# Avirup221/Multimodal-Hierarchical-CNN-for-Sun-Salutation-Pose-Classification

Measured on AMD Instinct MI355X. Metric: images/sec fwd+bwd QuadtreeCNN 224x224 bs256, higher is better.
Workload: dtype bf16; 1 GPU; QuadtreeCNN (ResNet-18 layer3, 2x2 split, 47-feat fusion) train step fwd+bwd+Adam, all parameters trainable; Adam(lr 1e-4, wd 1e-4) by the package's FusedAdam (csrc/pack.hip); global_batch=256, per_gpu_batch=256, image=3x224x224, num_classes=12, parallelism=dp1

## Files before the change

include/qtcnn.h:

```cpp
#ifndef QTCNN_H_
#define QTCNN_H_

#include <stddef.h>
#include <stdint.h>

#ifdef __cplusplus
extern "C" {
#endif

typedef enum qt_status {
  QT_OK = 0,
  QT_ERR_INVALID_ARG = -1,
  QT_ERR_LAUNCH = -2,
  QT_ERR_UNSUPPORTED = -3
} qt_status;

typedef enum qt_dtype { QT_F32 = 0, QT_BF16 = 1 } qt_dtype;

int qt_version(void);
const char* qt_last_error(void);

enum { QT_CONV_FWD = 0, QT_CONV_DGRAD = 1 };

typedef struct qt_conv_desc {
// ... 274 lines not shown
void qt_plan_destroy(qt_plan* plan);
int qt_plan_num_tensors(const qt_plan* plan);
const char* qt_plan_tensor_name(const qt_plan* plan, int i);
int qt_plan_tensor_kind(const qt_plan* plan, int i);
int qt_plan_tensor_shape(const qt_plan* plan, int i, int* dims4);
size_t qt_plan_workspace_bytes(const qt_plan* plan);
int qt_plan_find_buffer(const qt_plan* plan, const char* name, size_t* offset);
int qt_plan_profile_begin(qt_plan* plan);
int qt_plan_profile_end(qt_plan* plan, double* flops3, double* ms3, int* launches3);
int qt_plan_profile_bytes(const qt_plan* plan, double* bytes3);
int qt_plan_side_fence(qt_plan* plan, void* waiting_stream);
int qt_plan_init_workspace(qt_plan* plan, void* workspace, void* stream);
int qt_plan_pack_weights(qt_plan* plan, void* workspace, void* const* tensors, int for_backward, void* stream);
int qt_plan_adam_step(qt_plan* plan, void* workspace, void* const* tensors, float* const* grads, float* const* exp_avg,
                      float* const* exp_avg_sq, const qt_adam_desc* adam, int for_backward, void* stream);
int qt_plan_forward(qt_plan* plan, void* workspace, void* const* tensors, const float* image, const float* numerical,
                    float* logits, int batch, int training, unsigned long long seed, void* stream);
int qt_plan_backward(qt_plan* plan, void* workspace, void* const* tensors, float* const* grads, const float* numerical,
                     const float* dlogits, int phases, void* stream);
int qt_plan_backward_dx(qt_plan* plan, void* workspace, void* const* tensors, float* const* grads,
                        const float* numerical, const float* dlogits, int phases, float* dimage, void* stream);

#ifdef __cplusplus
}
#endif
#endif
```

multimodal-hierarchical-cnn-for-sun-salutation-pose-classification_amd/csrc/pack.hip:

```cpp
#include <math.h>
#include <string.h>

#include "qt_common.h"

namespace {

template <typename T> __device__ __forceinline__ T qt_from_f32(float v);
template <> __device__ __forceinline__ float qt_from_f32<float>(float v) { return v; }
template <> __device__ __forceinline__ bf16_t qt_from_f32<bf16_t>(float v) { return (bf16_t)v; }

template <typename T>
__global__ void pack_stem_input_kernel(const float* __restrict__ img, T* __restrict__ dst, int batch) {
  constexpr int PH = QT_STEM_PAD_H, PW = QT_STEM_PAD_W;
  const long long total = (long long)batch * PH * PW;
  for (long long i = blockIdx.x * (long long)blockDim.x + threadIdx.x; i < total;
       i += (long long)gridDim.x * blockDim.x) {
    const int pw = (int)(i % PW);
    const int ph = (int)((i / PW) % PH);
    const int n = (int)(i / ((long long)PW * PH));
    const int h = ph - 3, w = pw - 3;
    float v[4] = {0.f, 0.f, 0.f, 0.f};
    if ((unsigned)h < 224u && (unsigned)w < 224u) {
      const float* s = img + (long long)n * 3 * 224 * 224 + h * 224 + w;
      v[0] = s[0];
// ... 21 lines not shown
    const int o = (int)(idx / ((long long)I * taps));
    const float v = w[((long long)o * I + i) * taps + tap];
    if (fwd) fwd[idx] = qt_from_f32<T>(v);
    if (dgrad) dgrad[((long long)i * taps + tap) * O + o] = qt_from_f32<T>(v);
  }
}

struct AdamScalars {
  float lr, b1, b2, eps, wd;
  float step_size;
  float inv_sqrt_bc2;
  float grad_scale;
  int enabled;
};
__device__ __forceinline__ float adam_update(float p, float g, float& m, float& v, const AdamScalars& h) {
  g = g * h.grad_scale + h.wd * p;
  m = h.b1 * m + (1.f - h.b1) * g;
  v = h.b2 * v + (1.f - h.b2) * g * g;
  const float denom = sqrtf(v) * h.inv_sqrt_bc2 + h.eps;
  return p - h.step_size * (m / denom);
}

constexpr int PK_MAX_ITEMS = 32;
struct PackBatchArgs {
  AdamScalars adam;
  const float* g[PK_MAX_ITEMS];
  float* m[PK_MAX_ITEMS];
  float* v[PK_MAX_ITEMS];
  const float* w[PK_MAX_ITEMS];
  void* fwd[PK_MAX_ITEMS];
  void* dgrad[PK_MAX_ITEMS];
  int O[PK_MAX_ITEMS], I[PK_MAX_ITEMS];
  unsigned char k[PK_MAX_ITEMS], s2[PK_MAX_ITEMS];
  int first_block[PK_MAX_ITEMS + 1];
  int n;
};

template <typename T> struct PackPair;
template <> struct PackPair<float> {
  static __device__ __forceinline__ void store(float* p, float a, float b) { *reinterpret_cast<float2*>(p) = make_float2(a, b); }
};
template <> struct PackPair<bf16_t> {
  static __device__ __forceinline__ void store(bf16_t* p, float a, float b) {
    typedef __attribute__((ext_vector_type(2))) __bf16 bf16x2;
    bf16x2 v = {(bf16_t)a, (bf16_t)b};
    *reinterpret_cast<bf16x2*>(p) = v;
  }
};

template <typename T, int TAPS, int TO, int TI>
__device__ __forceinline__ void pack_tile(float* tile, const float* w, T* __restrict__ fwd, T* __restrict__ dg,
                                          int O, int I, int o0, int i0, int s2, const AdamScalars& adam,
                                          const float* __restrict__ g, float* m, float* v) {
  constexpr int RUN = TI * TAPS, S = RUN + 1, TOTAL = TO * RUN;
  for (int e = threadIdx.x; e < TOTAL; e += 256) {
    const int o = e / RUN, r = e - o * RUN;
    const long long idx = ((long long)(o0 + o) * I + i0) * TAPS + r;
    float pv = w[idx];
    if (adam.enabled) {
      float mv = m[idx], vv = v[idx];
      pv = adam_update(pv, g[idx], mv, vv, adam);
      m[idx] = mv;
      v[idx] = vv;
      const_cast<float*>(w)[idx] = pv;
    }
    tile[o * S + r] = pv;
  }
  __syncthreads();
  if (fwd) {
    for (int e = threadIdx.x; e < TOTAL / 2; e += 256) {
      const int i = (e % (TI / 2)) * 2, ot = e / (TI / 2);
      const int o = ot / TAPS, tap = ot - o * TAPS;
      const float* t = tile + o * S + i * TAPS + tap;
      PackPair<T>::store(fwd + ((long long)(o0 + o) * TAPS + tap) * I + i0 + i, t[0], t[TAPS]);
    }
  }
  if (dg) {
    for (int e = threadIdx.x; e < TOTAL / 2; e += 256) {
      const int o = (e % (TO / 2)) * 2, it2 = e / (TO / 2);
      const int i = it2 / TAPS, tap = it2 - i * TAPS;
      const float* t = tile + o * S + i * TAPS + tap;
      long long dst;
      if (TAPS == 1 && s2 == 4) {
        dst = ((long long)(i0 + i) * 5 + 4) * O + o0 + o;
      } else if (TAPS == 1 || !s2) {
        dst = ((long long)(i0 + i) * TAPS + tap) * O + o0 + o;
      } else {
        const int kh = tap / 3, kw = tap - kh * 3;
        const int ph = kh != 1, pw = kw != 1;
        const int th = ph ? (kh == 2 ? 0 : 1) : 0, tw = pw ? (kw == 2 ? 0 : 1) : 0;
        const int nh = ph ? 2 : 1, nw = pw ? 2 : 1;
        const int cls = ph * 2 + pw;
        const long long IO = (long long)I * O;
        const long long base = cls == 0 ? 0 : (cls == 1 ? IO : (cls == 2 ? 3 * IO : 5 * IO));
        dst = base + ((long long)(i0 + i) * (nh * nw) + th * nw + tw) * O + o0 + o;
        if (s2 == 2) dst = (((long long)cls * I + i0 + i) * 4 + th * 2 + tw) * O + o0 + o;
        if (s2 == 3) dst = (((long long)cls * I + i0 + i) * 5 + th * 2 + tw) * O + o0 + o;
      }
      PackPair<T>::store(dg + dst, t[0], t[S]);
    }
  }
}

constexpr int PK_T1 = 64;

template <typename T>
__global__ __launch_bounds__(256) void pack_weights_batched_kernel(PackBatchArgs a) {
  __shared__ float tile[32 * (32 * 9 + 1)];
  static_assert(PK_T1 * (PK_T1 + 1) <= 32 * (32 * 9 + 1), "1x1 tile fits the 3x3 tile's LDS");
  int it = 0;
  while (it + 1 < a.n && (int)blockIdx.x >= a.first_block[it + 1]) ++it;
  const int O = a.O[it], I = a.I[it];
  const int b = blockIdx.x - a.first_block[it];
  T* fwd = static_cast<T*>(a.fwd[it]);
  T* dg = static_cast<T*>(a.dgrad[it]);
  if (a.k[it] == 1) {
    const int tiles_i = I / PK_T1;
    pack_tile<T, 1, PK_T1, PK_T1>(tile, a.w[it], fwd, dg, O, I, (b / tiles_i) * PK_T1, (b % tiles_i) * PK_T1, (int)a.s2[it], a.adam,
                                  a.g[it], a.m[it], a.v[it]);
  } else {
    const int tiles_i = I >> 5;
    pack_tile<T, 9, 32, 32>(tile, a.w[it], fwd, dg, O, I, (b / tiles_i) << 5, (b % tiles_i) << 5, (int)a.s2[it], a.adam,
                            a.g[it], a.m[it], a.v[it]);
  }
}

constexpr int AD_MAX_ITEMS = 48, AD_CHUNK = 4096;
struct AdamBatchArgs {
  AdamScalars adam;
  float* p[AD_MAX_ITEMS];
  const float* g[AD_MAX_ITEMS];
  float* m[AD_MAX_ITEMS];
  float* v[AD_MAX_ITEMS];
  long long numel[AD_MAX_ITEMS];
  int first_block[AD_MAX_ITEMS + 1];
  int n;
};
__global__ __launch_bounds__(256) void adam_multi_kernel(AdamBatchArgs a) {
// ... 181 lines not shown
  QT_CHECK_ARG(items && n > 0 && n <= PK_MAX_ITEMS, "qt_pack_weights_batched: 1..%d items", PK_MAX_ITEMS);
  QT_CHECK_ARG(dtype == QT_F32 || dtype == QT_BF16, "qt_pack_weights_batched: bad dtype %d", dtype);
  PackBatchArgs a;
  memset(&a, 0, sizeof(a));
  if (opt) {
    if (int st = make_adam_scalars(adam, &a.adam)) return st;
  }
  int blocks = 0;
  for (int j = 0; j < n; ++j) {
    const qt_pack_item& q = items[j];
    const int te = q.k == 1 ? PK_T1 : 32;
    QT_CHECK_ARG(q.w_oihw && (q.w_fwd || q.w_dgrad) && (q.k == 1 || q.k == 3) && q.O > 0 && q.I > 0 && q.O % te == 0 &&
                     q.I % te == 0,
                 "qt_pack_weights_batched: item %d: O=%d I=%d must be multiples of %d for k=%d (k in {1,3})", j, q.O, q.I,
                 te, q.k);
    a.w[j] = q.w_oihw; a.fwd[j] = q.w_fwd; a.dgrad[j] = q.w_dgrad;
    if (opt) {
      const qt_adam_item& u = opt[j];
      QT_CHECK_ARG(u.param == q.w_oihw && u.grad && u.exp_avg && u.exp_avg_sq &&
                       u.numel == (long long)q.O * q.I * q.k * q.k,
                   "qt_adam_pack_weights_batched: item %d: optimizer state does not match the weight", j);
      a.g[j] = u.grad; a.m[j] = u.exp_avg; a.v[j] = u.exp_avg_sq;
    }
    a.O[j] = q.O; a.I[j] = q.I; a.k[j] = (unsigned char)q.k; a.s2[j] = (unsigned char)((q.stride2_dgrad >= 2 && q.stride2_dgrad <= 4) ? q.stride2_dgrad : (q.stride2_dgrad ? 1 : 0));
    QT_CHECK_ARG(q.stride2_dgrad != 4 || q.k == 1, "qt_pack_weights_batched: item %d: stride2_dgrad = 4 is for 1x1 filters", j);
    QT_CHECK_ARG(q.stride2_dgrad != 3 || q.k == 3, "qt_pack_weights_batched: item %d: stride2_dgrad = 3 is for 3x3 filters", j);
    a.first_block[j] = blocks;
    blocks += (q.O / te) * (q.I / te);
  }
  a.first_block[n] = blocks;
  a.n = n;
  hipStream_t s = static_cast<hipStream_t>(stream);
  if (dtype == QT_F32)
    hipLaunchKernelGGL(pack_weights_batched_kernel<float>, dim3(blocks), dim3(256), 0, s, a);
  else
    hipLaunchKernelGGL(pack_weights_batched_kernel<bf16_t>, dim3(blocks), dim3(256), 0, s, a);
  QT_CHECK_LAUNCH();
  return QT_OK;
}

extern "C" int qt_pack_dgrad_s2(int dtype, const float* w_oihw, void* dst, int O, int I, int k, long long* class_offset,
                                int* class_kh, int* class_kw, void* stream) {
  QT_CHECK_ARG(w_oihw && O > 0 && I > 0 && (k == 1 || k == 3), "qt_pack_dgrad_s2: bad argument");
// ... 73 lines not shown
```

multimodal-hierarchical-cnn-for-sun-salutation-pose-classification_amd/csrc/plan.hip:

```cpp
#include <stdlib.h>
#include <string.h>

#include <algorithm>
#include <string>
#include <vector>

#include "qt_common.h"

static bool merged_s2_enabled() {
  static int v = -1;
  if (v < 0) {
    const char* e = getenv("QTCNN_S2_DGRAD_MERGED");
    v = e ? (atoi(e) != 0) : 1;
  }
  return v != 0;
}

static bool ds_slot_enabled() {
  static int v = -1;
  if (v < 0) {
    const char* e = getenv("QTCNN_DS_SLOT");
    v = e ? (atoi(e) != 0) : 1;
  }
  return v != 0;
// ... 71 lines not shown
  size_t stats_bn2 = 0, stats_ds = 0, stats_bn1 = 0;
  size_t dw_begin = 0, dw_end = 0;
  size_t lin_ws = 0, lin_ws_bytes = 0;
  size_t wgrad_part = 0, wgrad_part_bytes = 0;
  bool packed_fwd = false, packed_bwd = false;
  unsigned long long packed_sig = 0;
  bool dw_dirty = true;
  int bwd_rows_bn2 = 0;
  struct Timed { hipEvent_t a, b; double flops; double bytes; int kind; };
  double last_profile_bytes[3] = {0, 0, 0};
  bool profiling = false;
  std::vector<Timed> timed;
  bool use_side = true;
  hipStream_t side = nullptr;
  hipEvent_t ev_fork = nullptr, ev_join = nullptr;
  int last_batch = 0, last_training = 0;
  unsigned long long last_seed = 0;

  int add_tensor(const std::string& name, int kind, std::initializer_list<int> shape) {
    TensorInfo t;
    t.name = name;
    t.kind = kind;
    t.ndim = (int)shape.size();
    int i = 0;
    for (int s : shape) t.shape[i++] = s;
    for (; i < 4; ++i) t.shape[i] = 1;
    tensors.push_back(t);
    return (int)tensors.size() - 1;
  }
  int add_bn(const std::string& prefix, int C) {
// ... 590 lines not shown
}
size_t dgrad_operand(const qt_plan* p, const ConvL& c) {
  return (c.k == 1 && c.slot_conv >= 0) ? p->convs[c.slot_conv].w_dgrad : c.w_dgrad;
}

unsigned long long weight_sig(const qt_plan* p, void* const* T) {
  unsigned long long h = 1469598103934665603ull;
  auto mix = [&](const void* ptr) { h = (h ^ (unsigned long long)(uintptr_t)ptr) * 1099511628211ull; };
  for (const ConvL& c : p->convs) mix(T[c.w]);
  mix(T[p->cls0.w]);
  return h;
}

int pack_weights(qt_plan* p, void* workspace, void* const* T, int for_backward, void* stream) {
  Exec e{p, static_cast<unsigned char*>(workspace), T, stream, p->d.batch, p->d.dtype};
  std::vector<qt_pack_item> items;
  auto add = [&](const float* w, void* fwd, void* dgrad, int O, int I, int k, int s2) {
    qt_pack_item q;
    q.w_oihw = w; q.w_fwd = fwd; q.w_dgrad = dgrad; q.O = O; q.I = I; q.k = k; q.stride2_dgrad = s2;
    items.push_back(q);
  };
  if (p->has_image) {
    for (size_t i = 0; i < p->convs.size(); ++i) {
      const ConvL& c = p->convs[i];
      if (i == 0)
        e.run(qt_pack_stem_weight(e.dt, e.tf(c.w), e.at(c.w_fwd), e.stem_taps(), stream));
      else
        add(e.tf(c.w), e.at(c.w_fwd), for_backward ? e.at(dgrad_operand(p, c)) : nullptr, c.cout, c.cin, c.k, dgrad_layout(c));
    }
  }
  if (!p->lstm)
    add(e.tf(p->cls0.w), e.at(p->cls0.w_fwd), for_backward ? e.at(p->cls0.w_dgrad) : nullptr, p->cls0.out, p->cls0.in, 1,
        false);
  for (size_t j = 0; j < items.size() && e.ok(); j += 32)
    e.run(qt_pack_weights_batched(e.dt, items.data() + j, (int)std::min<size_t>(32, items.size() - j), stream));
  p->packed_fwd = e.ok();
  p->packed_bwd = e.ok() && for_backward != 0;
  p->packed_sig = weight_sig(p, T);
  return e.status;
}

int adam_step(qt_plan* p, void* workspace, void* const* T, float* const* G, float* const* M1, float* const* M2,
              const qt_adam_desc* adam, int for_backward, void* stream) {
  Exec e{p, static_cast<unsigned char*>(workspace), T, stream, p->d.batch, p->d.dtype};
  std::vector<bool> fused(p->tensors.size(), false);
  std::vector<qt_pack_item> upd_items, pack_items;
  std::vector<qt_adam_item> upd_state, plain;
  auto numel_of = [&](int idx) {
    long long n = 1;
    for (int d = 0; d < p->tensors[idx].ndim; ++d) n *= p->tensors[idx].shape[d];
    return n;
  };
  auto add = [&](int widx, void* fwd, void* dgrad, int O, int I, int k, int s2) -> int {
    qt_pack_item q;
    q.w_oihw = e.tf(widx); q.w_fwd = fwd; q.w_dgrad = dgrad; q.O = O; q.I = I; q.k = k; q.stride2_dgrad = s2;
    if (G[widx]) {
      QT_CHECK_ARG(M1[widx] && M2[widx], "qt_plan_adam_step: %s has a gradient but no optimizer state",
                   p->tensors[widx].name.c_str());
      qt_adam_item u;
      u.param = e.tf(widx); u.grad = G[widx]; u.exp_avg = M1[widx]; u.exp_avg_sq = M2[widx]; u.numel = numel_of(widx);
      upd_items.push_back(q);
      upd_state.push_back(u);
// ... 5 lines not shown
  };
  if (p->has_image)
    for (size_t i = 1; i < p->convs.size(); ++i) {
      const ConvL& c = p->convs[i];
      if (int st = add(c.w, e.at(c.w_fwd), for_backward ? e.at(dgrad_operand(p, c)) : nullptr, c.cout, c.cin, c.k, dgrad_layout(c))) return st;
    }
  if (!p->lstm)
    if (int st = add(p->cls0.w, e.at(p->cls0.w_fwd), for_backward ? e.at(p->cls0.w_dgrad) : nullptr, p->cls0.out, p->cls0.in, 1, false))
      return st;
  for (size_t i = 0; i < p->tensors.size(); ++i) {
    if (p->tensors[i].kind != 0 || fused[i] || !G[i]) continue;
    QT_CHECK_ARG(T[i] && M1[i] && M2[i], "qt_plan_adam_step: %s has a gradient but no parameter / optimizer state",
                 p->tensors[i].name.c_str());
    qt_adam_item u;
    u.param = e.tf((int)i); u.grad = G[i]; u.exp_avg = M1[i]; u.exp_avg_sq = M2[i]; u.numel = numel_of((int)i);
    plain.push_back(u);
  }
  if (!plain.empty()) e.run(qt_adam_multi(plain.data(), (int)plain.size(), adam, stream));
  if (p->has_image)
    e.run(qt_pack_stem_weight(e.dt, e.tf(p->convs[0].w), e.at(p->convs[0].w_fwd), e.stem_taps(), stream));
  for (size_t j = 0; j < upd_items.size() && e.ok(); j += 32) {
    const int cnt = (int)std::min<size_t>(32, upd_items.size() - j);
    e.run(qt_adam_pack_weights_batched(e.dt, upd_items.data() + j, upd_state.data() + j, adam, cnt, stream));
  }
  const unsigned long long sig = weight_sig(p, T);
  const bool frozen_current = p->packed_fwd && (!for_backward || p->packed_bwd) && p->packed_sig == sig;
  if (!frozen_current)
    for (size_t j = 0; j < pack_items.size() && e.ok(); j += 32)
      e.run(qt_pack_weights_batched(e.dt, pack_items.data() + j, (int)std::min<size_t>(32, pack_items.size() - j), stream));
  p->packed_fwd = e.ok();
  p->packed_bwd = e.ok() && (for_backward != 0);
  p->packed_sig = sig;
  return e.status;
}

int forward(qt_plan* p, void* workspace, void* const* T, const float* image, const float* numerical, float* logits,
            int batch, int training, unsigned long long seed, void* stream) {
  Exec e{p, static_cast<unsigned char*>(workspace), T, stream, batch, p->d.dtype};
  e.setup_side();
  const int dt = e.dt;
  const bool tr = training == 1;
  const bool unf = training != 0;
  hipStream_t hs = static_cast<hipStream_t>(stream);
  auto quad_branch = [&]() {
    const ConvL& cq = p->convs[p->quad_conv];
    e.igemm(e.quad_desc(QT_CONV_FWD), e.at(p->blocks[5].out), e.at(cq.w_fwd), e.at(p->q), nullptr, e.tf(cq.bias),
            nullptr, nullptr, nullptr, 1);
    e.run(qt_quad_pool(dt, e.at(p->q), e.at(p->fused), batch, p->fused_ld, 512, e.stream));
  };
  auto mlp_branch = [&]() {
    qt_gemm_small_desc g;
    memset(&g, 0, sizeof(g));
    g.M = batch; g.N = p->mlp0.out; g.K = p->mlp0.in;
    g.a_dtype = QT_F32; g.b_dtype = QT_F32; g.c_dtype = QT_F32;
// ... 324 lines not shown
    qt_set_error("qt_plan_backward_dx: CnnLstm has no input gradient (its ResNet-18 is frozen and gradients through the "
                 "LSTM into the backbone are not implemented)");
    return QT_ERR_UNSUPPORTED;
  }
  if (dimage && p->has_image && p->last_training == 0) {
    qt_set_error("qt_plan_backward_dx: the last forward ran fused eval kernels (training = 0) and kept nothing for a "
                 "backward to the image; run it with training = 2 (eval statistics, tensors kept)");
    return QT_ERR_UNSUPPORTED;
  }
  QT_CHECK_ARG(!dimage || !p->has_image || p->packed_bwd,
               "qt_plan_backward_dx: the data-gradient operands are not packed (qt_plan_pack_weights with for_backward = 1)");
  Bwd e;
  e.p = p; e.ws = static_cast<unsigned char*>(workspace); e.T = T; e.stream = stream; e.B = p->last_batch;
  e.dt = p->d.dtype; e.G = G;
  e.setup_side();
  if ((phases & QT_BWD_HEAD) || p->dw_dirty) {
    e.run(zero(e.at(p->dw_begin), p->dw_end - p->dw_begin, stream));
    p->dw_dirty = false;
  }
  if (phases & QT_BWD_LAYER1) p->dw_dirty = true;
  const int dt = e.dt;
  const int B = e.B;
  const bool tr = p->last_training == 1;
  e.evalbn = p->last_training == 2;
  const float drop_mul = (tr && p->d.dropout_p > 0.f) ? 1.f / (1.f - p->d.dropout_p) : 1.f;
  bool backbone_grads = false;
  if (p->has_image)
    for (size_t i = 0; i < p->convs.size(); ++i) {
      if ((int)i == p->quad_conv || (int)i == p->sub_conv) continue;
      if (G[p->convs[i].w]) backbone_grads = true;
// ... 274 lines not shown
      if (bi == 0) rows_bn2 = 0;
    }
    p->bwd_rows_bn2 = rows_bn2;
    if (do_rest) {
    const ConvL& c0 = p->convs[0];
    const BnL& bn0 = p->bns[c0.bn];
    static const bool fused = !(getenv("QTCNN_STEM_FUSED") && atoi(getenv("QTCNN_STEM_FUSED")) == 0);
    bool stem_done = false;
    if (fused) {
      const int rows = qt_stem_bn_bwd_sums_rows(B);
      e.run(qt_stem_bn_bwd_sums(dt, e.at(p->g_p0), e.at(p->ymax), e.at<float>(bn0.scale), e.at<float>(bn0.shift),
                                e.at<float>(bn0.mean), e.at<float>(bn0.invstd), e.at<float>(p->stats), B, stream));
      e.run(qt_bn_bwd_finalize(e.at<float>(p->stats), rows, bn0.C, e.bn_count((long long)B * 112 * 112), e.tf(bn0.gamma),
                               e.at<float>(bn0.invstd), e.gf(bn0.gamma), e.gf(bn0.beta), 0, e.at<float>(bn0.coef), stream));
      if (e.gf(c0.w)) {
        e.fork();
        void* ws_ = e.wstream;
        const int slot = e.begin_timed(e.conv_flops(e.stem_desc(true)), 2, ws_, e.wgrad_bytes(c0, e.stem_desc(true)));
        const int st = qt_stem_bn_bwd_wgrad_ws(dt, e.at(p->g_p0), e.at<unsigned char>(p->argmax), e.at(c0.y),
                                               e.at<float>(bn0.scale), e.at<float>(bn0.shift), e.at<float>(bn0.mean),
                                               e.at<float>(bn0.invstd), e.at<float>(bn0.coef), e.at(p->xpad),
                                               e.at<float>(c0.dw), e.at(p->wgrad_part), p->wgrad_part_bytes, B, ws_);
        e.end_timed(slot, ws_);
        if (st == QT_OK) {
          e.run(qt_unpack_stem_wgrad(e.at<float>(c0.dw), e.gf(c0.w), 0, ws_));
          stem_done = true;
        } else if (st != QT_ERR_UNSUPPORTED) {
          e.run(st);
        }
      }
      if (!stem_done || want_dx)
        e.run(qt_stem_bn_bwd_apply(dt, e.at(p->g_p0), e.at<unsigned char>(p->argmax), e.at(c0.y), e.at<float>(bn0.scale),
                                   e.at<float>(bn0.shift), e.at<float>(bn0.mean), e.at<float>(bn0.invstd),
                                   e.at<float>(bn0.coef), e.at(c0.gy), B, stream));
    } else {
      e.run(qt_stem_pool_bwd(dt, e.at(p->g_p0), e.at<unsigned char>(p->argmax), e.at(c0.y), e.at<float>(bn0.scale),
                             e.at<float>(bn0.shift), e.at(c0.gy), B, stream));
      e.bn_backward(c0, e.at(c0.gy), nullptr);
    }
    if (!stem_done) e.wgrad(c0, e.stem_desc(true), e.at(p->xpad), true);
    if (want_dx) e.run(qt_stem_dgrad(dt, e.at(c0.gy), e.tf(c0.w), dimage, B, stream));
// ... 152 lines not shown
    qt_set_error("qt_plan_init_workspace: HIP error");
    return QT_ERR_LAUNCH;
  }
  return QT_OK;
}

extern "C" int qt_plan_pack_weights(qt_plan* p, void* workspace, void* const* tensors, int for_backward, void* stream) {
  QT_CHECK_ARG(p && workspace && tensors, "qt_plan_pack_weights: null argument");
  return pack_weights(p, workspace, tensors, for_backward, stream);
}

extern "C" int qt_plan_adam_step(qt_plan* p, void* workspace, void* const* tensors, float* const* grads,
                                 float* const* exp_avg, float* const* exp_avg_sq, const qt_adam_desc* adam, int for_backward,
                                 void* stream) {
  QT_CHECK_ARG(p && workspace && tensors && grads && exp_avg && exp_avg_sq && adam, "qt_plan_adam_step: null argument");
  return adam_step(p, workspace, tensors, grads, exp_avg, exp_avg_sq, adam, for_backward, stream);
}

extern "C" int qt_plan_forward(qt_plan* p, void* workspace, void* const* tensors, const float* image,
                               const float* numerical, float* logits, int batch, int training,
                               unsigned long long seed, void* stream) {
  QT_CHECK_ARG(p && workspace && tensors && logits, "qt_plan_forward: null argument");
  QT_CHECK_ARG(batch > 0 && batch <= p->d.batch, "qt_plan_forward: batch %d exceeds the plan's %d", batch, p->d.batch);
  QT_CHECK_ARG(!p->lstm || batch % p->seq_len == 0, "qt_plan_forward: %d frames are not whole sequences of %d", batch, p->seq_len);
  QT_CHECK_ARG(!p->has_image || image, "qt_plan_forward: image required");
  QT_CHECK_ARG(!p->has_numerical || numerical, "qt_plan_forward: numerical input required");
  QT_CHECK_ARG(((uintptr_t)workspace % 256) == 0, "qt_plan_forward: workspace must be 256-byte aligned");
  return forward(p, workspace, tensors, image, numerical, logits, batch, training, seed, stream);
}

extern "C" int qt_plan_backward(qt_plan* p, void* workspace, void* const* tensors, float* const* grads,
// ... 16 lines not shown
```

multimodal-hierarchical-cnn-for-sun-salutation-pose-classification_amd/engine.py:

```python
import ctypes
import os

import torch

from . import _lib
from ._lib import QtError

QT_MODEL_QUADTREE, QT_MODEL_STANDARD_RESNET, QT_MODEL_ATTENTION, QT_MODEL_CNN_LSTM = 0, 1, 2, 3
MODES = {"fusion": 0, "image_only": 1, "numerical_only": 2}
QT_BWD_HEAD, QT_BWD_LAYER4, QT_BWD_LAYER32, QT_BWD_LAYER1, QT_BWD_ALL = 1, 2, 4, 8, 15


class PlanDesc(ctypes.Structure):
    _fields_ = [
        ("dtype", ctypes.c_int), ("batch", ctypes.c_int), ("num_classes", ctypes.c_int),
        ("model", ctypes.c_int), ("mode", ctypes.c_int), ("numerical_dim", ctypes.c_int),
        ("dropout_p", ctypes.c_float), ("bn_eps", ctypes.c_float), ("bn_momentum", ctypes.c_float),
        ("seq_len", ctypes.c_int), ("lstm_hidden", ctypes.c_int),
    ]


def default_compute_dtype():
    name = os.environ.get("QTCNN_DTYPE", "bf16").lower()
    if name in ("bf16", "bfloat16"):
# ... 25 lines not shown
    L.qt_plan_tensor_kind.argtypes = [ctypes.c_void_p, ctypes.c_int]
    L.qt_plan_tensor_shape.argtypes = [ctypes.c_void_p, ctypes.c_int, ctypes.POINTER(ctypes.c_int)]
    L.qt_plan_workspace_bytes.argtypes = [ctypes.c_void_p]
    L.qt_plan_workspace_bytes.restype = ctypes.c_size_t
    L.qt_plan_init_workspace.argtypes = [ctypes.c_void_p, ctypes.c_void_p, ctypes.c_void_p]
    L.qt_plan_pack_weights.argtypes = [ctypes.c_void_p, ctypes.c_void_p, ctypes.c_void_p, ctypes.c_int, ctypes.c_void_p]
    L.qt_plan_forward.argtypes = [ctypes.c_void_p, ctypes.c_void_p, ctypes.c_void_p, ctypes.c_void_p, ctypes.c_void_p,
                                  ctypes.c_void_p, ctypes.c_int, ctypes.c_int, ctypes.c_ulonglong, ctypes.c_void_p]
    L.qt_plan_backward.argtypes = [ctypes.c_void_p, ctypes.c_void_p, ctypes.c_void_p, ctypes.c_void_p, ctypes.c_void_p,
                                   ctypes.c_void_p, ctypes.c_int, ctypes.c_void_p]
    L.qt_plan_backward_dx.argtypes = [ctypes.c_void_p, ctypes.c_void_p, ctypes.c_void_p, ctypes.c_void_p,
                                      ctypes.c_void_p, ctypes.c_void_p, ctypes.c_int, ctypes.c_void_p, ctypes.c_void_p]
    L.qt_plan_side_fence.argtypes = [ctypes.c_void_p, ctypes.c_void_p]
    L.qt_plan_adam_step.argtypes = [ctypes.c_void_p, ctypes.c_void_p, ctypes.c_void_p, ctypes.c_void_p, ctypes.c_void_p,
                                    ctypes.c_void_p, ctypes.POINTER(AdamDesc), ctypes.c_int, ctypes.c_void_p]
    L.qt_plan_find_buffer.argtypes = [ctypes.c_void_p, ctypes.c_char_p, ctypes.POINTER(ctypes.c_size_t)]
    L._plan_bound = True


class PlanEngine:

    def __init__(self, model_kind, mode, num_classes, numerical_dim, dropout_p, batch, dtype, device, seq_len=0,
                 lstm_hidden=0):
        self.L = _lib.lib()
        _bind_api(self.L)
        self.device = torch.device(device)
        if self.device.type != "cuda":
            raise QtError("the QuadtreeCNN plan runs on an AMD GPU only (device must be cuda:N); no CPU fallback")
        self.dtype = dtype
        self.max_batch = int(batch)
# ... 22 lines not shown
            self.shapes.append(tuple(dims[k] for k in range(nd)))
        self.index = {name: i for i, name in enumerate(self.names)}
        nbytes = self.L.qt_plan_workspace_bytes(handle)
        with torch.cuda.device(self.device):
            self.workspace = torch.empty(nbytes + 256, dtype=torch.uint8, device=self.device)
            off = (-self.workspace.data_ptr()) % 256
            self.ws_ptr = ctypes.c_void_p(self.workspace.data_ptr() + off)
            _lib.check(self.L.qt_plan_init_workspace(handle, self.ws_ptr, _lib.stream_ptr()), "qt_plan_init_workspace")
        self.workspace_bytes = nbytes
        self._tensor_ptrs = (ctypes.c_void_p * n)()
        self._packed_version = None
        self._weights_stale = True
        self.fwd_counter = 0
        self.grad_sync = None
        self._flat_grad = None

    @staticmethod
    def _storage_idle(t):
        try:
            return torch._C._storage_Use_Count(t.untyped_storage()._cdata) <= 2
        except Exception:
            return False

    def __del__(self):
        try:
            if getattr(self, "handle", None):
                self.L.qt_plan_destroy(self.handle)
                self.handle = None
        except Exception:
            pass
# ... 17 lines not shown
    def bind(self, tensors):
        for i, name in enumerate(self.names):
            t = tensors.get(name)
            if t is None:
                raise QtError(f"model is missing tensor {name!r} required by the plan")
            if tuple(t.shape) != self.shapes[i]:
                raise QtError(f"{name}: shape {tuple(t.shape)} != plan shape {self.shapes[i]}")
            want = torch.int64 if self.kinds[i] == 2 else torch.float32
            if t.dtype != want or t.device != self.device or not t.is_contiguous():
                raise QtError(f"{name}: expected contiguous {want} on {self.device}, got {t.dtype} on {t.device}")
            ptr = t.data_ptr()
            if self._tensor_ptrs[i] != ptr:
                self._weights_stale = True
            self._tensor_ptrs[i] = ptr

    def adam_step(self, by_index, desc):
        n = len(self.names)
        g, m, v = (ctypes.c_void_p * n)(), (ctypes.c_void_p * n)(), (ctypes.c_void_p * n)()
        for idx, (gt, mt, vt) in by_index.items():
            for t in (gt, mt, vt):
                if t.dtype != torch.float32 or t.device != self.device or not t.is_contiguous():
                    raise QtError(f"{self.names[idx]}: gradient / Adam state must be contiguous f32 on {self.device}")
            g[idx], m[idx], v[idx] = gt.data_ptr(), mt.data_ptr(), vt.data_ptr()
        _lib.check(self.L.qt_plan_adam_step(self.handle, self.ws_ptr, self._tensor_ptrs, g, m, v, ctypes.byref(desc), 1,
                                            _lib.stream_ptr()), "qt_plan_adam_step")
        self._weights_stale = False
        if self._packed_version is not None:
            self._packed_version = (self._packed_version[0], True)

    def invalidate_weights(self):
        self._weights_stale = True

    def pack_weights(self, version, for_backward):
        key = (version, bool(for_backward))
        if not self._weights_stale and self._packed_version is not None and self._packed_version[0] == version and \
                (self._packed_version[1] or not for_backward):
            return
        _lib.check(self.L.qt_plan_pack_weights(self.handle, self.ws_ptr, self._tensor_ptrs, int(for_backward),
                                               _lib.stream_ptr()), "qt_plan_pack_weights")
        self._packed_version = key
        self._weights_stale = False

    def forward(self, image, numerical, training, seed):
        batch = int(image.shape[0]) if image is not None else int(numerical.shape[0])
        logits = torch.empty(batch // self.rows_per_logit, self.num_classes, dtype=torch.float32, device=self.device)
        _lib.check(self.L.qt_plan_forward(self.handle, self.ws_ptr, self._tensor_ptrs,
                                          _lib.ptr(image), _lib.ptr(numerical), _lib.ptr(logits), batch,
                                          int(training), ctypes.c_ulonglong(seed), _lib.stream_ptr()),
                   "qt_plan_forward")
        self.fwd_counter += 1
        return logits

    @staticmethod
    def gradient_buckets(names, wanted):
        def bucket_of(idx):
            name = names[idx]
            if not name.startswith("base_cnn."):
                return 0
            if name.startswith("base_cnn.layer4."):
                return 1
            return 2 if name.startswith(("base_cnn.layer3.", "base_cnn.layer2.")) else 3
        order = sorted(wanted, key=lambda w: bucket_of(w[0]))
        sizes = {idx: int(torch.Size(shape).numel()) for idx, shape in wanted}
        offs, total, ends = {}, 0, [0, 0, 0, 0]
        for idx, _ in order:
# ... 19 lines not shown

        if wanted:
            self._weights_stale = True

        def run(phase):
            if dimage is None:
                _lib.check(self.L.qt_plan_backward(self.handle, self.ws_ptr, self._tensor_ptrs, grad_ptrs,
                                                   _lib.ptr(numerical), _lib.ptr(dlogits), phase, _lib.stream_ptr()),
                           "qt_plan_backward")
            else:
                _lib.check(self.L.qt_plan_backward_dx(self.handle, self.ws_ptr, self._tensor_ptrs, grad_ptrs,
                                                      _lib.ptr(numerical), _lib.ptr(dlogits), phase, _lib.ptr(dimage),
                                                      _lib.stream_ptr()),
                           "qt_plan_backward_dx")

        if self.grad_sync is None:
            run(QT_BWD_ALL)
        else:
            begin = 0
            for b, phase in enumerate((QT_BWD_HEAD, QT_BWD_LAYER4, QT_BWD_LAYER32, QT_BWD_LAYER1)):
                run(phase)
                if ends[b] > begin:
                    self.grad_sync(flat[begin:ends[b]], phase, self.side_fence)
                begin = ends[b]
            self.grad_sync(None, 0, None)
        return [views[idx] for idx, _ in wanted]


class PlanFunction(torch.autograd.Function):

    @staticmethod
    def forward(ctx, owner, image, numerical, *params):
# ... 38 lines not shown
```

multimodal-hierarchical-cnn-for-sun-salutation-pose-classification_amd/optim.py:

```python
import ctypes

import torch

from . import _lib
from .engine import AdamDesc, AdamItem


_raw_updates = 0


def raw_update_count():
    return _raw_updates


class FusedAdam(torch.optim.Optimizer):
    def __init__(self, params, lr=1e-3, betas=(0.9, 0.999), eps=1e-8, weight_decay=0.0, model=None):
        if lr < 0 or eps < 0 or weight_decay < 0 or not (0 <= betas[0] < 1) or not (0 <= betas[1] < 1):
            raise ValueError("FusedAdam: invalid hyper-parameters")
        super().__init__(params, dict(lr=lr, betas=betas, eps=eps, weight_decay=weight_decay))
        self._model = model

    @torch.no_grad()
    def step(self, closure=None):
        loss = None
        if closure is not None:
            with torch.enable_grad():
                loss = closure()
        engine = getattr(self._model, "_engine", None) if self._model is not None else None
        plan_index = {}
        if engine is not None and self._model._param_list is not None:
            plan_index = {id(p): i for p, i in zip(self._model._param_list, self._model._param_plan_index) if i >= 0}
        L = _lib.lib()
        L.qt_adam_multi.argtypes = [ctypes.POINTER(AdamItem), ctypes.c_int, ctypes.POINTER(AdamDesc), ctypes.c_void_p]
        fused_groups = 0
        for group in self.param_groups:
            todo = []
            for p in group["params"]:
                if p.grad is None:
                    continue
                if p.grad.is_sparse or p.dtype != torch.float32 or p.device.type != "cuda" or not p.is_contiguous():
                    raise _lib.QtError("FusedAdam handles dense contiguous f32 parameters on the GPU")
                st = self.state[p]
                if not st:
                    st["step"] = 0
                    st["exp_avg"] = torch.zeros_like(p, memory_format=torch.preserve_format)
                    st["exp_avg_sq"] = torch.zeros_like(p, memory_format=torch.preserve_format)
                st["step"] += 1
                todo.append((p, st))
            if not todo:
                continue
            steps = {st["step"] for _, st in todo}
            for step in sorted(steps):
                part = [(p, st) for p, st in todo if st["step"] == step]
                desc = AdamDesc(group["lr"], group["betas"][0], group["betas"][1], group["eps"], group["weight_decay"],
                                1.0, step)
                in_plan = {plan_index[id(p)]: (p.grad.contiguous(), st["exp_avg"], st["exp_avg_sq"])
                           for p, st in part if id(p) in plan_index}
                rest = [(p, st) for p, st in part if id(p) not in plan_index]
                if in_plan and engine is not None and fused_groups == 0 and len(steps) == 1 and \
                        len(self.param_groups) == 1:
                    with torch.cuda.device(engine.device):
                        engine.adam_step(in_plan, desc)
                    fused_groups += 1
                else:
                    rest = part
                    if engine is not None:
                        engine.invalidate_weights()
                if rest:
                    items = (AdamItem * len(rest))()
                    keep = []
                    for j, (p, st) in enumerate(rest):
                        g = p.grad.contiguous()
                        keep.append(g)
                        items[j] = AdamItem(p.data_ptr(), g.data_ptr(), st["exp_avg"].data_ptr(),
                                            st["exp_avg_sq"].data_ptr(), p.numel())
                    with torch.cuda.device(rest[0][0].device):
                        _lib.check(L.qt_adam_multi(items, len(rest), ctypes.byref(desc), _lib.stream_ptr()),
# ... 5 lines not shown
```

Before: 45650 images/s.

## Overlap fused Adam and weight packing with stem wgrad on a side stream

Moves the bulk Adam update and weight repacking onto the side stream so they can run concurrently with the stem weight-gradient kernel, which is moved onto the main stream for bf16 runs. Only the stem weight's Adam update stays on the main stream, and an event join makes the main stream wait for the side stream afterwards. The pack/Adam kernel is also changed to move data in float4 groups, stage tiles in T-typed LDS, and use smaller 3x3 tiles (16x32) to get more blocks. In exchange it adds stream-safety bookkeeping for handed-out gradients and a 16-byte alignment requirement on all pointers.

```diff
diff --git a/include/qtcnn.h b/include/qtcnn.h
--- a/include/qtcnn.h
+++ b/include/qtcnn.h
@@ -312,6 +312,9 @@
 int qt_plan_pack_weights(qt_plan* plan, void* workspace, void* const* tensors, int for_backward, void* stream);
 int qt_plan_adam_step(qt_plan* plan, void* workspace, void* const* tensors, float* const* grads, float* const* exp_avg,
                       float* const* exp_avg_sq, const qt_adam_desc* adam, int for_backward, void* stream);
+int qt_plan_adam_step_overlapped(qt_plan* plan, void* workspace, void* const* tensors, float* const* grads,
+                                 float* const* exp_avg, float* const* exp_avg_sq, const qt_adam_desc* adam, int for_backward,
+                                 void* stream, int* overlapped);
 int qt_plan_forward(qt_plan* plan, void* workspace, void* const* tensors, const float* image, const float* numerical,
                     float* logits, int batch, int training, unsigned long long seed, void* stream);
 int qt_plan_backward(qt_plan* plan, void* workspace, void* const* tensors, float* const* grads, const float* numerical,
diff --git a/multimodal-hierarchical-cnn-for-sun-salutation-pose-classification_amd/csrc/pack.hip b/multimodal-hierarchical-cnn-for-sun-salutation-pose-classification_amd/csrc/pack.hip
--- a/multimodal-hierarchical-cnn-for-sun-salutation-pose-classification_amd/csrc/pack.hip
+++ b/multimodal-hierarchical-cnn-for-sun-salutation-pose-classification_amd/csrc/pack.hip
@@ -1,4 +1,5 @@
 #include <math.h>
+#include <stdint.h>
 #include <string.h>
 
 #include "qt_common.h"
@@ -59,11 +60,13 @@
   int enabled;
 };
 __device__ __forceinline__ float adam_update(float p, float g, float& m, float& v, const AdamScalars& h) {
-  g = g * h.grad_scale + h.wd * p;
-  m = h.b1 * m + (1.f - h.b1) * g;
-  v = h.b2 * v + (1.f - h.b2) * g * g;
-  const float denom = sqrtf(v) * h.inv_sqrt_bc2 + h.eps;
-  return p - h.step_size * (m / denom);
+  g = __builtin_fmaf(h.wd, p, g * h.grad_scale);
+  m = __builtin_fmaf(h.b1, m, (1.f - h.b1) * g);
+  float v_old = h.b2 * v, v_new = (1.f - h.b2) * g * g;
+  asm("" : "+v"(v_old), "+v"(v_new));
+  v = v_old + v_new;
+  const float denom = __builtin_fmaf(sqrtf(v), h.inv_sqrt_bc2, h.eps);
+  return __builtin_fmaf(-h.step_size, m / denom, p);
 }
 
 constexpr int PK_MAX_ITEMS = 32;
@@ -81,50 +84,63 @@
   int n;
 };
 
-template <typename T> struct PackPair;
-template <> struct PackPair<float> {
-  static __device__ __forceinline__ void store(float* p, float a, float b) { *reinterpret_cast<float2*>(p) = make_float2(a, b); }
+template <typename T> struct PackQuad;
+template <> struct PackQuad<float> {
+  static __device__ __forceinline__ void store(float* p, float a, float b, float c, float d) {
+    *reinterpret_cast<float4*>(p) = make_float4(a, b, c, d);
+  }
 };
-template <> struct PackPair<bf16_t> {
-  static __device__ __forceinline__ void store(bf16_t* p, float a, float b) {
-    typedef __attribute__((ext_vector_type(2))) __bf16 bf16x2;
-    bf16x2 v = {(bf16_t)a, (bf16_t)b};
-    *reinterpret_cast<bf16x2*>(p) = v;
+template <> struct PackQuad<bf16_t> {
+  static __device__ __forceinline__ void store(bf16_t* p, bf16_t a, bf16_t b, bf16_t c, bf16_t d) {
+    bf16x4 v = {a, b, c, d};
+    *reinterpret_cast<bf16x4*>(p) = v;
   }
 };
 
 template <typename T, int TAPS, int TO, int TI>
-__device__ __forceinline__ void pack_tile(float* tile, const float* w, T* __restrict__ fwd, T* __restrict__ dg,
+__device__ __forceinline__ void pack_tile(T* tile, const float* w, T* __restrict__ fwd, T* __restrict__ dg,
                                           int O, int I, int o0, int i0, int s2, const AdamScalars& adam,
                                           const float* __restrict__ g, float* m, float* v) {
-  constexpr int RUN = TI * TAPS, S = RUN + 1, TOTAL = TO * RUN;
-  for (int e = threadIdx.x; e < TOTAL; e += 256) {
-    const int o = e / RUN, r = e - o * RUN;
+  constexpr int RUN = TI * TAPS, S = RUN + (TAPS == 1 ? 2 : 4), TOTAL = TO * RUN;
+  static_assert(RUN % 4 == 0 && TO % 4 == 0 && TI % 4 == 0, "tiles move in groups of four");
+#pragma unroll 1
+  for (int e = threadIdx.x; e < TOTAL / 4; e += 256) {
+    const int o = e / (RUN / 4), r = (e - o * (RUN / 4)) * 4;
     const long long idx = ((long long)(o0 + o) * I + i0) * TAPS + r;
-    float pv = w[idx];
+    float4 pv = *reinterpret_cast<const float4*>(w + idx);
     if (adam.enabled) {
-      float mv = m[idx], vv = v[idx];
-      pv = adam_update(pv, g[idx], mv, vv, adam);
-      m[idx] = mv;
-      v[idx] = vv;
-      const_cast<float*>(w)[idx] = pv;
-    }
-    tile[o * S + r] = pv;
+      float4 gv = *reinterpret_cast<const float4*>(g + idx);
+      float4 mv = *reinterpret_cast<const float4*>(m + idx), vv = *reinterpret_cast<const float4*>(v + idx);
+      pv.x = adam_update(pv.x, gv.x, mv.x, vv.x, adam);
+      asm volatile("" : "+v"(pv.x), "+v"(gv.y));
+      pv.y = adam_update(pv.y, gv.y, mv.y, vv.y, adam);
+      asm volatile("" : "+v"(pv.y), "+v"(gv.z));
+      pv.z = adam_update(pv.z, gv.z, mv.z, vv.z, adam);
+      asm volatile("" : "+v"(pv.z), "+v"(gv.w));
+      pv.w = adam_update(pv.w, gv.w, mv.w, vv.w, adam);
+      *reinterpret_cast<float4*>(m + idx) = mv;
+      *reinterpret_cast<float4*>(v + idx) = vv;
+      *reinterpret_cast<float4*>(const_cast<float*>(w) + idx) = pv;
+    }
+    T* t = tile + o * S + r;
+    t[0] = qt_from_f32<T>(pv.x); t[1] = qt_from_f32<T>(pv.y); t[2] = qt_from_f32<T>(pv.z); t[3] = qt_from_f32<T>(pv.w);
   }
   __syncthreads();
   if (fwd) {
-    for (int e = threadIdx.x; e < TOTAL / 2; e += 256) {
-      const int i = (e % (TI / 2)) * 2, ot = e / (TI / 2);
+#pragma unroll 1
+    for (int e = threadIdx.x; e < TOTAL / 4; e += 256) {
+      const int i = (e % (TI / 4)) * 4, ot = e / (TI / 4);
       const int o = ot / TAPS, tap = ot - o * TAPS;
-      const float* t = tile + o * S + i * TAPS + tap;
-      PackPair<T>::store(fwd + ((long long)(o0 + o) * TAPS + tap) * I + i0 + i, t[0], t[TAPS]);
+      const T* t = tile + o * S + i * TAPS + tap;
+      PackQuad<T>::store(fwd + ((long long)(o0 + o) * TAPS + tap) * I + i0 + i, t[0], t[TAPS], t[2 * TAPS], t[3 * TAPS]);
     }
   }
   if (dg) {
-    for (int e = threadIdx.x; e < TOTAL / 2; e += 256) {
-      const int o = (e % (TO / 2)) * 2, it2 = e / (TO / 2);
+#pragma unroll 1
+    for (int e = threadIdx.x; e < TOTAL / 4; e += 256) {
+      const int o = (e % (TO / 4)) * 4, it2 = e / (TO / 4);
       const int i = it2 / TAPS, tap = it2 - i * TAPS;
-      const float* t = tile + o * S + i * TAPS + tap;
+      const T* t = tile + o * S + i * TAPS + tap;
       long long dst;
       if (TAPS == 1 && s2 == 4) {
         dst = ((long long)(i0 + i) * 5 + 4) * O + o0 + o;
@@ -142,17 +158,18 @@
         if (s2 == 2) dst = (((long long)cls * I + i0 + i) * 4 + th * 2 + tw) * O + o0 + o;
         if (s2 == 3) dst = (((long long)cls * I + i0 + i) * 5 + th * 2 + tw) * O + o0 + o;
       }
-      PackPair<T>::store(dg + dst, t[0], t[S]);
-    }
-  }
-}
-
-constexpr int PK_T1 = 64;
+      PackQuad<T>::store(dg + dst, t[0], t[S], t[2 * S], t[3 * S]);
+    }
+  }
+}
+
+constexpr int PK_T1 = 64, PK_T3O = 16, PK_T3I = 32;
+constexpr int PK_TILE_ELEMS = PK_T3O * (PK_T3I * 9 + 4);
 
 template <typename T>
 __global__ __launch_bounds__(256) void pack_weights_batched_kernel(PackBatchArgs a) {
-  __shared__ float tile[32 * (32 * 9 + 1)];
-  static_assert(PK_T1 * (PK_T1 + 1) <= 32 * (32 * 9 + 1), "1x1 tile fits the 3x3 tile's LDS");
+  __shared__ __attribute__((aligned(16))) T tile[PK_TILE_ELEMS];
+  static_assert(PK_T1 * (PK_T1 + 2) <= PK_TILE_ELEMS, "1x1 tile fits the 3x3 tile's LDS");
   int it = 0;
   while (it + 1 < a.n && (int)blockIdx.x >= a.first_block[it + 1]) ++it;
   const int O = a.O[it], I = a.I[it];
@@ -164,9 +181,9 @@
     pack_tile<T, 1, PK_T1, PK_T1>(tile, a.w[it], fwd, dg, O, I, (b / tiles_i) * PK_T1, (b % tiles_i) * PK_T1, (int)a.s2[it], a.adam,
                                   a.g[it], a.m[it], a.v[it]);
   } else {
-    const int tiles_i = I >> 5;
-    pack_tile<T, 9, 32, 32>(tile, a.w[it], fwd, dg, O, I, (b / tiles_i) << 5, (b % tiles_i) << 5, (int)a.s2[it], a.adam,
-                            a.g[it], a.m[it], a.v[it]);
+    const int tiles_i = I / PK_T3I;
+    pack_tile<T, 9, PK_T3O, PK_T3I>(tile, a.w[it], fwd, dg, O, I, (b / tiles_i) * PK_T3O, (b % tiles_i) * PK_T3I, (int)a.s2[it],
+                                    a.adam, a.g[it], a.m[it], a.v[it]);
   }
 }
 
@@ -378,6 +395,10 @@
                      q.I % te == 0,
                  "qt_pack_weights_batched: item %d: O=%d I=%d must be multiples of %d for k=%d (k in {1,3})", j, q.O, q.I,
                  te, q.k);
+    auto al16 = [](const void* x) { return (reinterpret_cast<uintptr_t>(x) & 15) == 0; };
+    QT_CHECK_ARG(al16(q.w_oihw) && al16(q.w_fwd) && al16(q.w_dgrad) &&
+                     (!opt || (al16(opt[j].grad) && al16(opt[j].exp_avg) && al16(opt[j].exp_avg_sq))),
+                 "qt_pack_weights_batched: item %d: every pointer must be 16-byte aligned", j);
     a.w[j] = q.w_oihw; a.fwd[j] = q.w_fwd; a.dgrad[j] = q.w_dgrad;
     if (opt) {
       const qt_adam_item& u = opt[j];
@@ -390,7 +411,7 @@
     QT_CHECK_ARG(q.stride2_dgrad != 4 || q.k == 1, "qt_pack_weights_batched: item %d: stride2_dgrad = 4 is for 1x1 filters", j);
     QT_CHECK_ARG(q.stride2_dgrad != 3 || q.k == 3, "qt_pack_weights_batched: item %d: stride2_dgrad = 3 is for 3x3 filters", j);
     a.first_block[j] = blocks;
-    blocks += (q.O / te) * (q.I / te);
+    blocks += q.k == 1 ? (q.O / PK_T1) * (q.I / PK_T1) : (q.O / PK_T3O) * (q.I / PK_T3I);
   }
   a.first_block[n] = blocks;
   a.n = n;
diff --git a/multimodal-hierarchical-cnn-for-sun-salutation-pose-classification_amd/csrc/plan.hip b/multimodal-hierarchical-cnn-for-sun-salutation-pose-classification_amd/csrc/plan.hip
--- a/multimodal-hierarchical-cnn-for-sun-salutation-pose-classification_amd/csrc/plan.hip
+++ b/multimodal-hierarchical-cnn-for-sun-salutation-pose-classification_amd/csrc/plan.hip
@@ -109,6 +109,7 @@
   bool use_side = true;
   hipStream_t side = nullptr;
   hipEvent_t ev_fork = nullptr, ev_join = nullptr;
+  bool tail_ready = false;
   int last_batch = 0, last_training = 0;
   unsigned long long last_seed = 0;
 
@@ -729,6 +730,7 @@
 
 int pack_weights(qt_plan* p, void* workspace, void* const* T, int for_backward, void* stream) {
   Exec e{p, static_cast<unsigned char*>(workspace), T, stream, p->d.batch, p->d.dtype};
+  p->tail_ready = false;
   std::vector<qt_pack_item> items;
   auto add = [&](const float* w, void* fwd, void* dgrad, int O, int I, int k, int s2) {
     qt_pack_item q;
@@ -756,11 +758,15 @@
 }
 
 int adam_step(qt_plan* p, void* workspace, void* const* T, float* const* G, float* const* M1, float* const* M2,
-              const qt_adam_desc* adam, int for_backward, void* stream) {
+              const qt_adam_desc* adam, int for_backward, void* stream, bool overlap, int* overlapped) {
   Exec e{p, static_cast<unsigned char*>(workspace), T, stream, p->d.batch, p->d.dtype};
+  const bool ov = overlap && p->tail_ready && p->use_side && p->side != nullptr && p->has_image;
+  p->tail_ready = false;
+  if (overlapped) *overlapped = ov;
+  void* bulk = ov ? static_cast<void*>(p->side) : stream;
   std::vector<bool> fused(p->tensors.size(), false);
   std::vector<qt_pack_item> upd_items, pack_items;
-  std::vector<qt_adam_item> upd_state, plain;
+  std::vector<qt_adam_item> upd_state, plain, stem_w;
   auto numel_of = [&](int idx) {
     long long n = 1;
     for (int d = 0; d < p->tensors[idx].ndim; ++d) n *= p->tensors[idx].shape[d];
@@ -796,20 +802,25 @@
                  p->tensors[i].name.c_str());
     qt_adam_item u;
     u.param = e.tf((int)i); u.grad = G[i]; u.exp_avg = M1[i]; u.exp_avg_sq = M2[i]; u.numel = numel_of((int)i);
-    plain.push_back(u);
-  }
-  if (!plain.empty()) e.run(qt_adam_multi(plain.data(), (int)plain.size(), adam, stream));
+    (ov && (int)i == p->convs[0].w ? stem_w : plain).push_back(u);
+  }
+  if (!plain.empty() && e.ok()) e.run(qt_adam_multi(plain.data(), (int)plain.size(), adam, bulk));
+  if (!stem_w.empty() && e.ok()) e.run(qt_adam_multi(stem_w.data(), 1, adam, stream));
   if (p->has_image)
     e.run(qt_pack_stem_weight(e.dt, e.tf(p->convs[0].w), e.at(p->convs[0].w_fwd), e.stem_taps(), stream));
   for (size_t j = 0; j < upd_items.size() && e.ok(); j += 32) {
     const int cnt = (int)std::min<size_t>(32, upd_items.size() - j);
-    e.run(qt_adam_pack_weights_batched(e.dt, upd_items.data() + j, upd_state.data() + j, adam, cnt, stream));
+    e.run(qt_adam_pack_weights_batched(e.dt, upd_items.data() + j, upd_state.data() + j, adam, cnt, bulk));
   }
   const unsigned long long sig = weight_sig(p, T);
   const bool frozen_current = p->packed_fwd && (!for_backward || p->packed_bwd) && p->packed_sig == sig;
   if (!frozen_current)
     for (size_t j = 0; j < pack_items.size() && e.ok(); j += 32)
-      e.run(qt_pack_weights_batched(e.dt, pack_items.data() + j, (int)std::min<size_t>(32, pack_items.size() - j), stream));
+      e.run(qt_pack_weights_batched(e.dt, pack_items.data() + j, (int)std::min<size_t>(32, pack_items.size() - j), bulk));
+  if (ov) {
+    (void)hipEventRecord(p->ev_join, p->side);
+    (void)hipStreamWaitEvent(static_cast<hipStream_t>(stream), p->ev_join, 0);
+  }
   p->packed_fwd = e.ok();
   p->packed_bwd = e.ok() && (for_backward != 0);
   p->packed_sig = sig;
@@ -820,6 +831,7 @@
             int batch, int training, unsigned long long seed, void* stream) {
   Exec e{p, static_cast<unsigned char*>(workspace), T, stream, batch, p->d.dtype};
   e.setup_side();
+  p->tail_ready = false;
   const int dt = e.dt;
   const bool tr = training == 1;
   const bool unf = training != 0;
@@ -1174,6 +1186,7 @@
   e.p = p; e.ws = static_cast<unsigned char*>(workspace); e.T = T; e.stream = stream; e.B = p->last_batch;
   e.dt = p->d.dtype; e.G = G;
   e.setup_side();
+  p->tail_ready = false;
   if ((phases & QT_BWD_HEAD) || p->dw_dirty) {
     e.run(zero(e.at(p->dw_begin), p->dw_end - p->dw_begin, stream));
     p->dw_dirty = false;
@@ -1478,8 +1491,15 @@
       e.run(qt_bn_bwd_finalize(e.at<float>(p->stats), rows, bn0.C, e.bn_count((long long)B * 112 * 112), e.tf(bn0.gamma),
                                e.at<float>(bn0.invstd), e.gf(bn0.gamma), e.gf(bn0.beta), 0, e.at<float>(bn0.coef), stream));
       if (e.gf(c0.w)) {
-        e.fork();
-        void* ws_ = e.wstream;
+        const bool on_main = dt == QT_BF16 && !want_dx && e.wstream != stream;
+        if (on_main) {
+          e.forked = true;
+          e.join();
+          e.fork();
+        } else {
+          e.fork();
+        }
+        void* ws_ = on_main ? stream : e.wstream;
         const int slot = e.begin_timed(e.conv_flops(e.stem_desc(true)), 2, ws_, e.wgrad_bytes(c0, e.stem_desc(true)));
         const int st = qt_stem_bn_bwd_wgrad_ws(dt, e.at(p->g_p0), e.at<unsigned char>(p->argmax), e.at(c0.y),
                                                e.at<float>(bn0.scale), e.at<float>(bn0.shift), e.at<float>(bn0.mean),
@@ -1489,6 +1509,7 @@
         if (st == QT_OK) {
           e.run(qt_unpack_stem_wgrad(e.at<float>(c0.dw), e.gf(c0.w), 0, ws_));
           stem_done = true;
+          p->tail_ready = on_main && e.ok() && (phases & QT_BWD_ALL) == QT_BWD_ALL;
         } else if (st != QT_ERR_UNSUPPORTED) {
           e.run(st);
         }
@@ -1671,7 +1692,14 @@
                                  float* const* exp_avg, float* const* exp_avg_sq, const qt_adam_desc* adam, int for_backward,
                                  void* stream) {
   QT_CHECK_ARG(p && workspace && tensors && grads && exp_avg && exp_avg_sq && adam, "qt_plan_adam_step: null argument");
-  return adam_step(p, workspace, tensors, grads, exp_avg, exp_avg_sq, adam, for_backward, stream);
+  return adam_step(p, workspace, tensors, grads, exp_avg, exp_avg_sq, adam, for_backward, stream, false, nullptr);
+}
+
+extern "C" int qt_plan_adam_step_overlapped(qt_plan* p, void* workspace, void* const* tensors, float* const* grads,
+                                            float* const* exp_avg, float* const* exp_avg_sq, const qt_adam_desc* adam,
+                                            int for_backward, void* stream, int* overlapped) {
+  QT_CHECK_ARG(p && workspace && tensors && grads && exp_avg && exp_avg_sq && adam, "qt_plan_adam_step_overlapped: null argument");
+  return adam_step(p, workspace, tensors, grads, exp_avg, exp_avg_sq, adam, for_backward, stream, true, overlapped);
 }
 
 extern "C" int qt_plan_forward(qt_plan* p, void* workspace, void* const* tensors, const float* image,
diff --git a/multimodal-hierarchical-cnn-for-sun-salutation-pose-classification_amd/engine.py b/multimodal-hierarchical-cnn-for-sun-salutation-pose-classification_amd/engine.py
--- a/multimodal-hierarchical-cnn-for-sun-salutation-pose-classification_amd/engine.py
+++ b/multimodal-hierarchical-cnn-for-sun-salutation-pose-classification_amd/engine.py
@@ -63,6 +63,7 @@
     L.qt_plan_side_fence.argtypes = [ctypes.c_void_p, ctypes.c_void_p]
     L.qt_plan_adam_step.argtypes = [ctypes.c_void_p, ctypes.c_void_p, ctypes.c_void_p, ctypes.c_void_p, ctypes.c_void_p,
                                     ctypes.c_void_p, ctypes.POINTER(AdamDesc), ctypes.c_int, ctypes.c_void_p]
+    L.qt_plan_adam_step_overlapped.argtypes = L.qt_plan_adam_step.argtypes + [ctypes.POINTER(ctypes.c_int)]
     L.qt_plan_find_buffer.argtypes = [ctypes.c_void_p, ctypes.c_char_p, ctypes.POINTER(ctypes.c_size_t)]
     L._plan_bound = True
 
@@ -115,6 +116,8 @@
         self.fwd_counter = 0
         self.grad_sync = None
         self._flat_grad = None
+        self._handed_out = None
+        self.last_adam_overlapped = False
 
     @staticmethod
     def _storage_idle(t):
@@ -162,7 +165,18 @@
                 self._weights_stale = True
             self._tensor_ptrs[i] = ptr
 
-    def adam_step(self, by_index, desc):
+    def adam_overlap_ok(self, by_index):
+        h = self._handed_out
+        if h is None or self.grad_sync is not None:
+            return False
+        flat, version, ptrs = h
+        if flat is not self._flat_grad or flat._version != version or set(by_index) != set(ptrs):
+            return False
+        return all(by_index[idx][0].data_ptr() == ptr for idx, ptr in ptrs.items())
+
+    def adam_step(self, by_index, desc, overlap=False):
+        overlap = bool(overlap) and self.adam_overlap_ok(by_index)
+        self._handed_out = None
         n = len(self.names)
         g, m, v = (ctypes.c_void_p * n)(), (ctypes.c_void_p * n)(), (ctypes.c_void_p * n)()
         for idx, (gt, mt, vt) in by_index.items():
@@ -170,8 +184,15 @@
                 if t.dtype != torch.float32 or t.device != self.device or not t.is_contiguous():
                     raise QtError(f"{self.names[idx]}: gradient / Adam state must be contiguous f32 on {self.device}")
             g[idx], m[idx], v[idx] = gt.data_ptr(), mt.data_ptr(), vt.data_ptr()
-        _lib.check(self.L.qt_plan_adam_step(self.handle, self.ws_ptr, self._tensor_ptrs, g, m, v, ctypes.byref(desc), 1,
-                                            _lib.stream_ptr()), "qt_plan_adam_step")
+        took = ctypes.c_int(0)
+        if overlap:
+            _lib.check(self.L.qt_plan_adam_step_overlapped(self.handle, self.ws_ptr, self._tensor_ptrs, g, m, v,
+                                                           ctypes.byref(desc), 1, _lib.stream_ptr(), ctypes.byref(took)),
+                       "qt_plan_adam_step_overlapped")
+        else:
+            _lib.check(self.L.qt_plan_adam_step(self.handle, self.ws_ptr, self._tensor_ptrs, g, m, v, ctypes.byref(desc), 1,
+                                                _lib.stream_ptr()), "qt_plan_adam_step")
+        self.last_adam_overlapped = bool(took.value)
         self._weights_stale = False
         if self._packed_version is not None:
             self._packed_version = (self._packed_version[0], True)
@@ -197,6 +218,7 @@
                                           int(training), ctypes.c_ulonglong(seed), _lib.stream_ptr()),
                    "qt_plan_forward")
         self.fwd_counter += 1
+        self._handed_out = None
         return logits
 
     @staticmethod
@@ -246,8 +268,11 @@
                                                       _lib.stream_ptr()),
                            "qt_plan_backward_dx")
 
+        self._handed_out = None
         if self.grad_sync is None:
             run(QT_BWD_ALL)
+            if dimage is None:
+                self._handed_out = (flat, flat._version, {idx: int(grad_ptrs[idx]) for idx, _ in wanted})
         else:
             begin = 0
             for b, phase in enumerate((QT_BWD_HEAD, QT_BWD_LAYER4, QT_BWD_LAYER32, QT_BWD_LAYER1)):
diff --git a/multimodal-hierarchical-cnn-for-sun-salutation-pose-classification_amd/optim.py b/multimodal-hierarchical-cnn-for-sun-salutation-pose-classification_amd/optim.py
--- a/multimodal-hierarchical-cnn-for-sun-salutation-pose-classification_amd/optim.py
+++ b/multimodal-hierarchical-cnn-for-sun-salutation-pose-classification_amd/optim.py
@@ -1,4 +1,5 @@
 import ctypes
+import os
 
 import torch
 
@@ -11,6 +12,14 @@
 
 def raw_update_count():
     return _raw_updates
+
+
+def overlap_allowed(engine, by_index, created_state, n_groups, n_steps):
+    if os.environ.get("QTCNN_ADAM_OVERLAP", "1") == "0":
+        return False
+    if created_state or n_groups != 1 or n_steps != 1:
+        return False
+    return engine is not None and engine.adam_overlap_ok(by_index)
 
 
 class FusedAdam(torch.optim.Optimizer):
@@ -35,6 +44,7 @@
         fused_groups = 0
         for group in self.param_groups:
             todo = []
+            created_state = False
             for p in group["params"]:
                 if p.grad is None:
                     continue
@@ -43,6 +53,7 @@
                 st = self.state[p]
                 if not st:
                     st["step"] = 0
+                    created_state = True
                     st["exp_avg"] = torch.zeros_like(p, memory_format=torch.preserve_format)
                     st["exp_avg_sq"] = torch.zeros_like(p, memory_format=torch.preserve_format)
                 st["step"] += 1
@@ -60,7 +71,8 @@
                 if in_plan and engine is not None and fused_groups == 0 and len(steps) == 1 and \
                         len(self.param_groups) == 1:
                     with torch.cuda.device(engine.device):
-                        engine.adam_step(in_plan, desc)
+                        engine.adam_step(in_plan, desc, overlap=overlap_allowed(
+                            engine, in_plan, created_state, len(self.param_groups), len(steps)))
                     fused_groups += 1
                 else:
                     rest = part
```

Measured after the change: 46720 images/s (median of 6 runs). 1.02x the previous value.
